# Terence-23/RayTracing-in-a-weekend

Measured on AMD Instinct MI355X. Metric: Msamples/s (rays x bounces) at 1920x1080x500spp, higher is better.
Workload: dtype f32

## Files before the change

raytracing-in-a-weekend_amd/csrc/rtw_host.cpp:

```cpp
#include "rtw_host.h"

#include <algorithm>
#include <cfloat>
#include <cmath>
#include <cstring>
#include <limits>

static_assert(sizeof(RtwCamera) == 84 && sizeof(RtwSphere) == 80 && sizeof(RtwTexture) == 16 && sizeof(RtwQuad) == 88, "POD layout");
static_assert(sizeof(RtwInstance) == 48 && sizeof(RtwScene) == 96 && sizeof(RtwParams) == 72 && sizeof(RtwStats) == 160, "POD layout");

namespace rtw {

uint32_t sampler_count(uint32_t sampler, uint32_t samples, uint32_t *s_root) {
    uint32_t root = 0, n = samples;
    if (sampler == RTW_SAMPLER_STRATIFIED) { root = (uint32_t)std::ceil(std::sqrt((float)samples)); n = root * root; }
    else if (sampler == RTW_SAMPLER_CENTRES) { root = (uint32_t)std::floor(std::sqrt((float)samples)); n = root * root; }
    else if (sampler == RTW_SAMPLER_NO_RAND) n = 1;
    if (s_root) *s_root = root;
    return n;
}

namespace {

struct V { float x, y, z; };
// ... 748 lines not shown
            if (!(radii[i] >= 16.0f * r_med) && std::isfinite(radii[i])) break;
            is_big[i] = 1; out.big.push_back(i);
        }
    }
    std::sort(out.big.begin(), out.big.end());

    Builder b;
    Box centres; box_empty(centres);
    float rmin = FLT_MAX, rmax = 0.0f;
    for (uint32_t i = 0; i < n; i++) {
        if (is_big[i]) continue;
        const RtwSphere &s = spheres[i];
        Prim p; p.sphere = i;
        for (int k = 0; k < 3; k++) {
            float c0 = s.center[k] + s.velocity[k] * t_begin;
            float c1 = s.center[k] + s.velocity[k] * t_end;
            float lo = std::min(c0, c1), hi = std::max(c0, c1);
            if (!(lo == lo) || !(hi == hi)) { lo = -FLT_MAX; hi = FLT_MAX; }
            centres.lo[k] = std::min(centres.lo[k], lo); centres.hi[k] = std::max(centres.hi[k], hi);
            p.cen[k] = 0.5f * lo + 0.5f * hi;
            if (!std::isfinite(p.cen[k])) p.cen[k] = 0.0f;
            p.box.lo[k] = std::nextafter(lo - radii[i], -FLT_MAX);
            p.box.hi[k] = std::nextafter(hi + radii[i], FLT_MAX);
        }
        rmin = std::min(rmin, radii[i]); rmax = std::max(rmax, radii[i]);
        b.prims.push_back(p);
    }
    if (b.prims.empty()) return;
    const uint32_t nl = (uint32_t)b.prims.size();
    Box root_box; box_empty(root_box);
    for (const Prim &p : b.prims) box_grow(root_box, p.box);
    float box_abs = 0.0f;
    for (int k = 0; k < 3; k++) box_abs = std::max(box_abs, std::max(std::fabs(root_box.lo[k]), std::fabs(root_box.hi[k])));
    const bool lds_candidate = nl >= 2 && nl - 1 <= RTW_LDS_NODES_MAX && n <= RTW_LDS_GEOM_MAX && box_abs < 30000.0f;
    b.cap = out.depth_cap = opt.depth_cap ? std::max(opt.depth_cap, ceil_log2(nl)) : bvh_depth_cap(nl, n, lds_candidate);
    b.sweep = opt.sweep && nl <= RTW_BVH_OPTIMISE_MAX;
    b.t.resize(nl);
    for (uint32_t i = 0; i < nl; i++) { b.t[i].box = b.prims[i].box; b.t[i].parent = -1; b.t[i].c[0] = b.t[i].c[1] = -1; b.t[i].height = 0; }
    b.t.reserve(2 * (size_t)nl);
    int32_t troot = b.build(0, nl, 0);
    for (uint32_t i = 0; i < nl; i++) b.t[i].box = b.prims[i].box;
    for (int32_t i = (int32_t)b.t.size() - 1; i >= (int32_t)nl; i--) b.refit(i);
    if (opt.reinsert && nl > 2 && nl <= RTW_BVH_OPTIMISE_MAX) b.reinsertion(troot);
    out.nodes.reserve(nl - 1);
    out.root = b.flatten(troot, 0, out.nodes, out.depth);
    double r2 = 0.0;
    for (int k = 0; k < 3; k++) {
        out.centre[k] = 0.5f * centres.lo[k] + 0.5f * centres.hi[k];
        double h = std::max(std::fabs((double)centres.hi[k] - out.centre[k]), std::fabs((double)centres.lo[k] - out.centre[k]));
        r2 += h * h;
        out.abs_max = std::max(out.abs_max, std::max(std::fabs(root_box.lo[k]), std::fabs(root_box.hi[k])));
    }
    out.centre_radius = (float)(std::sqrt(r2) * 1.000001);
    out.r_min = rmin; out.r_max = rmax;

    if (!out.nodes.empty() && out.nodes.size() <= RTW_LDS_NODES_MAX && n <= RTW_LDS_GEOM_MAX && out.abs_max < 30000.0f) {
        out.nodes16.resize(out.nodes.size());
        for (size_t i = 0; i < out.nodes.size(); i++) {
            const BvhNode &a = out.nodes[i]; BvhNode16 &b = out.nodes16[i];
            for (int k = 0; k < 3; k++) {
                b.plane[0][k][0] = half_bits(a.lo0[k], false); b.plane[0][k][1] = half_bits(a.hi0[k], true);
                b.plane[1][k][0] = half_bits(a.lo1[k], false); b.plane[1][k][1] = half_bits(a.hi1[k], true);
            }
            b.c0 = (int16_t)(a.c0 >= 0 ? a.c0 * 32 : a.c0); b.c1 = (int16_t)(a.c1 >= 0 ? a.c1 * 32 : a.c1); b.pad = 0;
        }
    }
}

void pack_nodes32(const std::vector<BvhNode16> &nodes16, std::vector<uint32_t> &out) {
    const uint32_t AX = RTW_NODE32_AXIS_DWORDS, ND = RTW_NODE32_DWORDS;
    out.assign(nodes16.size() * ND, 0u);
    auto widen = [](uint16_t h) { _Float16 v; std::memcpy(&v, &h, 2); const float f = (float)v; uint32_t u; std::memcpy(&u, &f, 4); return u; };
    auto code = [](int16_t c) { return (uint32_t)(uint16_t)(c >= 0 ? (c / 32) * (int)RTW_NODE32_CODE : (int)c); };
    for (size_t i = 0; i < nodes16.size(); i++) {
        const BvhNode16 &a = nodes16[i];
        uint32_t *d = out.data() + i * ND;
        for (int c = 0; c < 2; c++) for (int k = 0; k < 3; k++) {
            const uint32_t lo = widen(a.plane[c][k][0]), hi = widen(a.plane[c][k][1]);
            uint32_t *q = d + (size_t)(c * 3 + k) * AX;
            q[0] = hi; q[1] = lo; q[2] = lo; q[3] = hi;
        }
        const uint32_t cc = code(a.c0) | (code(a.c1) << 16);
        d[6u * AX] = cc; d[6u * AX + RTW_NODE32_OFF / 4u] = cc;
    }
}

}

namespace rtw {
namespace {
inline float half_value(uint16_t x) { _Float16 v; std::memcpy(&v, &x, 2); return (float)v; }
inline void host_sphere(const RtwSphere &s, uint32_t idx, const float o[3], const float d[3], float tm, float a, float mint, float maxt, int32_t &best, float &best_t) {
    float oc[3];
    for (int k = 0; k < 3; k++) oc[k] = o[k] - (s.center[k] + s.velocity[k] * tm);
    const float b = oc[0] * d[0] + oc[1] * d[1] + oc[2] * d[2], c = (oc[0] * oc[0] + oc[1] * oc[1] + oc[2] * oc[2]) - s.radius * s.radius;
    const float disc = b * b - a * c;
    if (!(disc >= 0.0f)) return;
    const float sq = std::sqrt(disc);
    float x = (-b - sq) / a;
    if (x < mint || x > maxt) x = (-b + sq) / a;
    if (x < mint || x > maxt) return;
    if (best < 0 || x < best_t || (x == best_t && (int32_t)idx < best)) { best = (int32_t)idx; best_t = x; }
}
}

HostHit bvh_closest_host(const BvhBuild &bb, const RtwSphere *spheres, uint32_t n, const float o[3], const float d[3], float tm,
                         float mint, float maxt, bool use_tree, std::string *ops) {
    HostHit h; h.sphere = -1; h.t = maxt; h.node_visits = h.leaf_tests = 0;
    const float a = d[0] * d[0] + d[1] * d[1] + d[2] * d[2];
    if (!use_tree) { for (uint32_t i = 0; i < n; i++) host_sphere(spheres[i], i, o, d, tm, a, mint, maxt, h.sphere, h.t); return h; }
    for (uint32_t i : bb.big) host_sphere(spheres[i], i, o, d, tm, a, mint, maxt, h.sphere, h.t);
    if (bb.root == std::numeric_limits<int32_t>::min()) return h;
    const float M = (std::fabs(o[0] - bb.centre[0]) + std::fabs(o[1] - bb.centre[1]) + std::fabs(o[2] - bb.centre[2])) * 1.0001f + bb.centre_radius;
    const float q = (M * M + bb.r_max * bb.r_max) * 1.4305115e-6f;
    const float sq_q = std::sqrt(q) * 1.0001f;
    float rho = std::fmin(q * (bb.r_min > 0.0f ? 1.0f / (2.0f * bb.r_min) : FLT_MAX), sq_q);
    rho = rho * 1.0001f + 4.8e-7f * (std::fabs(o[0]) + std::fabs(o[1]) + std::fabs(o[2]) + bb.abs_max);
    const float tau = sq_q * 1.0002f / std::sqrt(a) + 1e-30f;
    float inv[3], kp[3], km[3];
    for (int k = 0; k < 3; k++) {
        inv[k] = std::fabs(d[k]) >= 1e-20f ? 1.0f / d[k] : std::copysign(1e20f, d[k]);
        kp[k] = -(o[k] + rho) * inv[k]; km[k] = -(o[k] - rho) * inv[k];
    }
    const float lo_lim = mint - tau;
    const bool f16 = !bb.nodes16.empty();
    std::vector<int32_t> stack; stack.reserve(RTW_BVH_STACK + 2);
    int32_t node = bb.root;
    for (;;) {
        if (node >= 0) {
            h.node_visits++; if (ops) ops->push_back('N');
            const BvhNode &nd = bb.nodes[(size_t)node];
            float e[2], x[2];
            for (int c = 0; c < 2; c++) {
                e[c] = -FLT_MAX; x[c] = FLT_MAX;
                for (int k = 0; k < 3; k++) {
                    const float lo = f16 ? half_value(bb.nodes16[(size_t)node].plane[c][k][0]) : (c ? nd.lo1[k] : nd.lo0[k]);
                    const float hi = f16 ? half_value(bb.nodes16[(size_t)node].plane[c][k][1]) : (c ? nd.hi1[k] : nd.hi0[k]);
                    const float t1 = std::fma(lo, inv[k], kp[k]), t2 = std::fma(hi, inv[k], km[k]);
                    e[c] = std::fmax(e[c], std::fmin(t1, t2)); x[c] = std::fmin(x[c], std::fmax(t1, t2));
                }
            }
            const float hi_lim = h.t + tau;
            const float m0 = std::fmax(e[0], lo_lim), m1 = std::fmax(e[1], lo_lim);
            const bool h0 = m0 <= std::fmin(x[0], hi_lim), h1 = m1 <= std::fmin(x[1], hi_lim);
            if (h0 && h1) { const bool near0 = m0 <= m1; stack.push_back(near0 ? nd.c1 : nd.c0); node = near0 ? nd.c0 : nd.c1; continue; }
            if (h0 || h1) { node = h0 ? nd.c0 : nd.c1; continue; }
        } else {
            h.leaf_tests++; if (ops) ops->push_back('L');
            const uint32_t s = (uint32_t)~node;
            if (s < n) host_sphere(spheres[s], s, o, d, tm, a, mint, maxt, h.sphere, h.t);
        }
        if (stack.empty()) break;
        node = stack.back(); stack.pop_back();
    }
    return h;
}
}

extern "C" int rtw_bvh_dump(const RtwScene *sc, float t_begin, float t_end, void *nodes, uint32_t node_cap, uint32_t *n_nodes, int32_t *root,
                            uint32_t *depth, uint32_t *depth_cap, uint32_t *big, uint32_t big_cap, uint32_t *n_big, uint16_t *nodes16) {
    using namespace rtw;
    if (!sc || (sc->n_spheres && !sc->spheres)) return RTW_E_INVALID;
    BvhBuild b;
    build_bvh(sc->spheres, sc->n_spheres, t_begin, t_end, b);
    if (n_nodes) *n_nodes = (uint32_t)b.nodes.size();
    if (root) *root = b.root;
// ... 213 lines not shown
```

raytracing-in-a-weekend_amd/csrc/rtw_kernels.hip:

```cpp
#include "rtw_kernels.h"
#include "rtw_mesh.h"
#include <type_traits>

#ifndef RTW_MAX_TRIPS
#define RTW_MAX_TRIPS 0x30000000u
#endif

namespace rtw {


constexpr bool gradient_spec(int spec) { return spec >= 1 && spec <= 3; }
constexpr bool generic_spec(int spec) { return spec == 0 || spec == 7 || spec == 8 || spec == 9 || spec == 10 || spec == 11 || spec == 12; }
constexpr bool light_spec(int spec) { return spec == 9 || spec == 10 || spec == 11; }
constexpr int mixed_spec(int spec) { return spec == 10 ? 1 : spec == 11 ? 2 : 0; }
constexpr bool quat_spec(int spec) { return spec == 11; }
constexpr bool noise_spec(int spec) { return spec == 7; }
constexpr bool tri_spec(int spec) { return spec == 8 || spec == 12; }
constexpr bool mesh_spec(int spec) { return spec == 12; }
template <int SPEC> __device__ __forceinline__ uint32_t integ(const KArgs &A) {
    return (SPEC == 5 || SPEC == 12) ? (uint32_t)RTW_INTEGRATOR_RUST2 : SPEC == 4 ? (uint32_t)RTW_INTEGRATOR_BG_COLOR : !generic_spec(SPEC) ? (uint32_t)RTW_INTEGRATOR_GRADIENT : A.integrator;
}
template <int SPEC> __device__ __forceinline__ uint32_t samp(const KArgs &A) {
    return SPEC == 6 ? (uint32_t)RTW_SAMPLER_STRATIFIED : SPEC == 5 ? (uint32_t)RTW_SAMPLER_CENTRES : !generic_spec(SPEC) ? (uint32_t)RTW_SAMPLER_ROW : A.sampler;
}
// ... 592 lines not shown
            if (MOVING) { w0 = vel[s + 4]; w1 = vel[s + 5]; w2 = vel[s + 6]; w3 = vel[s + 7]; }
        }
        test(g0, v0, s); test(g1, v1, s + 1); test(g2, v2, s + 2); test(g3, v3, s + 3);
    }
    for (; s < n; ++s) test(geom[s], MOVING ? vel[s] : zero, s);
}

#ifndef RTW_GEOM_BRUTE_WAVES
#define RTW_GEOM_BRUTE_WAVES 4
#endif
template <bool MOVING, int SPEC, bool GEOM>
__global__ __launch_bounds__(RTW_BLOCK, GEOM ? RTW_GEOM_BRUTE_WAVES : 1) void render_brute(const KArgs A) {
    bool dead = false, have = false, newpath = false;
    Pixel px; px.ij = px.rng_base = px.s = px.slot = 0;
    Reserve rs; rs.next = rs.end = rs.limit = rs.i0 = rs.k0 = rs.s0 = rs.s1 = rs.slot0 = rs.tries = 0; rs.sub = blockIdx.x & ((1u << A.sub_shift) - 1u);
#ifdef RTW_ENDTIMES
    rs.t_dry = 0ull;
#endif
    Path pt; pt.o = pt.d = pt.L = mk(0, 0, 0); pt.thr = mk(1, 1, 1); pt.tm = 0; pt.k = 0; pt.poison = false; pt.rng.state = 0; pt.rng.inc = 1;
    uint32_t n_seg = 0, n_rays = 0, n_isph = 0, n_quad = 0;
    uint32_t trips = 0; bool aborted = false;
    if constexpr (tri_spec(SPEC)) tri_nodes_begin(A);

    for (;;) {
        if (fetch_pixel(A, !have && !dead, px, dead, rs)) { have = true; newpath = true; }
        if (ballot64(!dead) == 0ull) break;
        if (++trips > RTW_MAX_TRIPS) { aborted = true; break; }
        if (have && newpath) { newpath = false; start_path<SPEC>(A, px, pt); n_rays++; }
        if (have) {
            bool finished;
            if (light_spec(SPEC) ? (A.depth == 0 && (mixed_spec(SPEC) ? A.integrator != RTW_INTEGRATOR_LIGHT_CAST : A.integrator == RTW_INTEGRATOR_LIGHT_BIASED))
                                 : (generic_spec(SPEC) && A.depth == 0 && A.integrator != RTW_INTEGRATOR_NORMAL)) {
                pt.L = (light_spec(SPEC) || A.integrator == RTW_INTEGRATOR_RUST2) ? ld3(A.bg) : mk(0, 0, 0); finished = true;
            } else {
                int best; float best_t;
                closest_brute<MOVING>(A.sc, pt.o, pt.d, pt.tm, A.mint, A.maxt, best, best_t);
                n_seg++;
                if constexpr (light_spec(SPEC)) finished = light_step_brute<MOVING, GEOM, mixed_spec(SPEC), quat_spec(SPEC)>(A, pt, best, best_t, n_seg, n_isph, n_quad);
                else finished = GEOM ? shade_geom<MOVING, SPEC>(A, pt, best, best_t, n_isph, n_quad) : shade<MOVING, SPEC>(A, pt, best, best_t);
            }
            if (finished) {
                if (finish_path<SPEC>(A, px, pt)) have = false;
                else newpath = true;
            }
        }
    }
    if constexpr (tri_spec(SPEC)) tri_nodes_end(A);
    flush_counters(A, n_seg, n_rays, (unsigned long long)n_seg * A.sc.n + n_isph, 0);
    if (GEOM) flush_quads(A, n_quad);
    if (aborted && (threadIdx.x & 63u) == 0) atomicAdd(&A.stats[23], 1ull);
}


template <bool MOVING>
__device__ __forceinline__ void exact_sphere(f4 g, f4 vv, uint32_t s, v3 o, v3 d, float tm, float a, float ra, bool a_plain, float mint, float maxt,
                                             int &best, float &best_t) {
    float cx = g.x, cy = g.y, cz = g.z;
    if (MOVING) { cx = cx + vv.x * tm; cy = cy + vv.y * tm; cz = cz + vv.z * tm; }
    float ocx = o.x - cx, ocy = o.y - cy, ocz = o.z - cz;
    float b = ocx * d.x + ocy * d.y + ocz * d.z;
    float c = (ocx * ocx + ocy * ocy + ocz * ocz) - g.w;
    float disc = b * b - a * c;
    if (!(disc < 0.0f)) {
        const float x = sphere_root(b, disc, a, ra, a_plain, mint);
        const bool take = !(x < mint || x > maxt) && (x < best_t || (x == best_t && s < (uint32_t)best));
        best = take ? (int)s : best; best_t = take ? x : best_t;
    }
}

#define RTW_KU 1.4305115e-6f
#ifndef RTW_S_HI
#define RTW_S_HI 52u
#endif
#ifndef RTW_TRAV_UNROLL
#define RTW_TRAV_UNROLL 3
#endif
#ifndef RTW_T_LO
#define RTW_T_LO 6u
#endif
#ifndef RTW_T_LO_DRAIN
#define RTW_T_LO_DRAIN RTW_T_LO
#endif

struct Trav {
    int node;
    uint32_t sp;
    int best; float best_t;
    float a, ra;
    float ix, iy, iz;
    float kpx, kpy, kpz;
    float kmx, kmy, kmz;
    uint32_t selx, sely, selz;
    float tau_t, lo_lim, hi_lim;
};

template <class S> struct Code;
template <> struct Code<short> { enum : int { END = 0x7FFF, DEAD = 0x7FFE }; };
template <> struct Code<int> { enum : int { END = 0x7FFFFFFF, DEAD = 0x7FFFFFFE }; };
template <class S> __device__ __forceinline__ bool in_trav(int node) { return (uint32_t)node < (uint32_t)Code<S>::DEAD; }
template <class S> __device__ __forceinline__ bool in_leaf(int node) { return (uint32_t)node > (uint32_t)Code<S>::END; }
template <class S> __device__ __forceinline__ uint32_t leaf_sphere(int node) { return (uint32_t)node ^ (sizeof(S) == 2 ? 0xFFFFu : 0xFFFFFFFFu); }
template <class S> __device__ __forceinline__ bool in_shade(int node) { return node == (int)Code<S>::END; }

__device__ __forceinline__ uint32_t lanes_in(bool c) {
    uint32_t n = (uint32_t)__popcll(ballot64(c));
    asm volatile("" : "+s"(n));
    return n;
}

struct BvhBegin {
    const f4 *big_geom; const f4 *big_vel; const uint32_t *big_index;
    uint32_t n_big, depth; int32_t root;
    float cx, cy, cz, centre_radius, r_max2, inv_2rmin, abs_max;
};
static_assert(sizeof(BvhBegin) == 64 && offsetof(DevBvh, abs_max) - offsetof(DevBvh, big_geom) == 60 && offsetof(DevBvh, big_vel) == offsetof(DevBvh, big_geom) + 8 &&
              offsetof(DevBvh, n_big) == offsetof(DevBvh, big_geom) + 24 && offsetof(DevBvh, root) == offsetof(DevBvh, big_geom) + 32 &&
              offsetof(DevBvh, cx) == offsetof(DevBvh, big_geom) + 36, "BvhBegin mirrors DevBvh from big_geom on");
__device__ __forceinline__ BvhBegin load_bvh_begin() {
    typedef uint32_t u16v __attribute__((ext_vector_type(16)));
    u16v r;
    asm volatile("s_load_dwordx16 %0, %1, %2\n\ts_waitcnt lgkmcnt(0)" : "=s"(r) : "s"(__builtin_amdgcn_kernarg_segment_ptr()),
                 "n"(offsetof(KArgs, bvh) + offsetof(DevBvh, big_geom)));
    BvhBegin b;
    b.big_geom = (const f4 *)(uintptr_t)((uint64_t)r[0] | ((uint64_t)r[1] << 32));
    b.big_vel = (const f4 *)(uintptr_t)((uint64_t)r[2] | ((uint64_t)r[3] << 32));
    b.big_index = (const uint32_t *)(uintptr_t)((uint64_t)r[4] | ((uint64_t)r[5] << 32));
    b.n_big = r[6]; b.depth = r[7]; b.root = (int32_t)r[8];
    b.cx = __uint_as_float(r[9]); b.cy = __uint_as_float(r[10]); b.cz = __uint_as_float(r[11]); b.centre_radius = __uint_as_float(r[12]);
    b.r_max2 = __uint_as_float(r[13]); b.inv_2rmin = __uint_as_float(r[14]); b.abs_max = __uint_as_float(r[15]);
    return b;
}

template <class T> __device__ __forceinline__ T lds_get(uint32_t addr) { return *(const __attribute__((address_space(3))) T *)(uintptr_t)addr; }
template <class T> __device__ __forceinline__ void lds_put(uint32_t addr, T v) { *(__attribute__((address_space(3))) T *)(uintptr_t)addr = v; }
__device__ __forceinline__ uint32_t lds_addr(const void *p) { return (uint32_t)(uintptr_t)(const __attribute__((address_space(3))) void *)p; }

template <bool MOVING, class S, bool F32 = false>
__device__ __forceinline__ void trav_begin(const KArgs &A, const Path &pt, Trav &tr, uint32_t sp0, bool a_plain_wave, bool &a_odd, Cen *cn = nullptr) {
    RTW_CEN(cn, CEN_TRAV_BEGIN);
    const BvhBegin bv = load_bvh_begin();
    const v3 o = pt.o, d = pt.d;
    tr.a = dot(d, d);
    tr.ra = rcp_refined(tr.a);
    a_odd = !in_range(tr.a, 0x1p-20f, 0x1p20f);
    const bool a_plain = a_plain_wave && ballot64(a_odd) == 0ull;
    tr.best = -1; tr.best_t = A.maxt; tr.sp = sp0;
    {
        cf4_ptr bg = (cf4_ptr)(uintptr_t)bv.big_geom;
        cf4_ptr bvel = (cf4_ptr)(uintptr_t)bv.big_vel;
        typedef const uint32_t __attribute__((address_space(4))) *cu32_ptr;
        cu32_ptr bidx = (cu32_ptr)(uintptr_t)bv.big_index;
        for (uint32_t k = 0; k < bv.n_big; ++k) {
            f4 vv = MOVING ? bvel[k] : f4{ 0, 0, 0, 0 };
            exact_sphere<MOVING>(bg[k], vv, bidx[k], o, d, pt.tm, tr.a, tr.ra, a_plain, A.mint, A.maxt, tr.best, tr.best_t);
        }
    }
    if (bv.root == (int)0x80000000) { tr.node = (int)Code<S>::END; return; }
    tr.node = sizeof(S) == 2 ? (bv.root >= 0 ? bv.root * (F32 ? (int)RTW_NODE32_CODE : 32) : (int)((uint32_t)bv.root & 0xFFFFu)) : bv.root;
    const float ex = o.x - bv.cx, ey = o.y - bv.cy, ez = o.z - bv.cz;
#ifdef RTW_BEGIN_L2_NORM
    const float M = __builtin_amdgcn_sqrtf(ex * ex + ey * ey + ez * ez) * 1.0001f + bv.centre_radius;
#else
    const float M = (__builtin_fabsf(ex) + __builtin_fabsf(ey) + __builtin_fabsf(ez)) * 1.0001f + bv.centre_radius;
#endif
    const float q = (M * M + bv.r_max2) * RTW_KU;
    const float sq_q = __builtin_amdgcn_sqrtf(q) * 1.0001f;
    float rho = fminf(q * bv.inv_2rmin, sq_q);
    rho = rho * 1.0001f + 4.8e-7f * (fabsf(o.x) + fabsf(o.y) + fabsf(o.z) + bv.abs_max);
    tr.tau_t = sq_q * 1.0002f * __builtin_amdgcn_rsqf(tr.a) + 1e-30f;
    float ix = __builtin_amdgcn_rcpf(d.x), iy = __builtin_amdgcn_rcpf(d.y), iz = __builtin_amdgcn_rcpf(d.z);
#ifdef RTW_BEGIN_GUARD_PER_LANE
    if (!(fabsf(d.x) >= 1e-20f)) ix = copysignf(1e20f, d.x);
    if (!(fabsf(d.y) >= 1e-20f)) iy = copysignf(1e20f, d.y);
    if (!(fabsf(d.z) >= 1e-20f)) iz = copysignf(1e20f, d.z);
#else
    if (ballot64(!(fminf(fminf(fabsf(d.x), fabsf(d.y)), fabsf(d.z)) >= 1e-20f) || d.x != d.x || d.y != d.y || d.z != d.z) != 0ull) {
        if (!(fabsf(d.x) >= 1e-20f)) ix = copysignf(1e20f, d.x);
        if (!(fabsf(d.y) >= 1e-20f)) iy = copysignf(1e20f, d.y);
        if (!(fabsf(d.z) >= 1e-20f)) iz = copysignf(1e20f, d.z);
    }
#endif
    tr.ix = ix; tr.iy = iy; tr.iz = iz;
    if (sizeof(S) == 2) {
        const float ox = -o.x * ix, oy = -o.y * iy, oz = -o.z * iz;
        const float rx = rho * fabsf(ix), ry = rho * fabsf(iy), rz = rho * fabsf(iz);
        tr.kpx = ox - rx; tr.kpy = oy - ry; tr.kpz = oz - rz;
        tr.kmx = ox + rx; tr.kmy = oy + ry; tr.kmz = oz + rz;
        const uint32_t ID = 0x03020100u, FLIP = 0x03020100u ^ 0x01000302u;
        if (F32) {
            tr.selx = ~(uint32_t)((int32_t)__float_as_uint(ix) >> 31) & RTW_NODE32_OFF;
            tr.sely = ~(uint32_t)((int32_t)__float_as_uint(iy) >> 31) & RTW_NODE32_OFF;
            tr.selz = ~(uint32_t)((int32_t)__float_as_uint(iz) >> 31) & RTW_NODE32_OFF;
        } else {
        tr.selx = ID ^ ((uint32_t)((int32_t)__float_as_uint(ix) >> 31) & FLIP);
        tr.sely = ID ^ ((uint32_t)((int32_t)__float_as_uint(iy) >> 31) & FLIP);
        tr.selz = ID ^ ((uint32_t)((int32_t)__float_as_uint(iz) >> 31) & FLIP);
        }
    } else {
        tr.kpx = -(o.x + rho) * ix; tr.kpy = -(o.y + rho) * iy; tr.kpz = -(o.z + rho) * iz;
        tr.kmx = -(o.x - rho) * ix; tr.kmy = -(o.y - rho) * iy; tr.kmz = -(o.z - rho) * iz;
    }
    tr.lo_lim = A.mint - tr.tau_t;
    tr.hi_lim = tr.best_t + tr.tau_t;
}


template <class S, uint32_t BLOCK = RTW_BLOCK>
__device__ __forceinline__ void trav_pop(Trav &tr) {
    tr.node = (int)(uint32_t)lds_get<typename std::make_unsigned<S>::type>(tr.sp);
    tr.sp -= BLOCK * (uint32_t)sizeof(S);
}

template <class S> __device__ __forceinline__ int entry_to_node(uint32_t raw);
template <> __device__ __forceinline__ int entry_to_node<short>(uint32_t raw) { return (int)(raw & 0xFFFFu); }
template <> __device__ __forceinline__ int entry_to_node<int>(uint32_t raw) { return (int)raw; }

template <class S, uint32_t BLOCK = RTW_BLOCK>
__device__ __forceinline__ void trav_descend(Trav &tr, float e0, float x0, float e1, float x1,
                                             uint32_t c0, uint32_t c1, uint32_t popped) {
    const float n0 = fmaxf(e0, tr.lo_lim), n1 = fmaxf(e1, tr.lo_lim);
    const bool h0 = n0 <= fminf(x0, tr.hi_lim);
    const bool h1 = n1 <= fminf(x1, tr.hi_lim);
    const bool le = n0 <= n1;
    const bool both = h0 && h1, none = !(h0 || h1);
    const bool near0 = h0 && (!h1 || le);
    const uint32_t level = BLOCK * (uint32_t)sizeof(S);
    if (sizeof(S) == 2) {
        const uint64_t H0 = __builtin_amdgcn_ballot_w64(h0), H1 = __builtin_amdgcn_ballot_w64(h1), LE = __builtin_amdgcn_ballot_w64(le);
        const bool far0 = __builtin_amdgcn_inverse_ballot_w64(~H0 | (H1 & ~LE));
        const uint32_t nf = __builtin_amdgcn_alignbit(c0, c0, far0 ? 16u : 0u);
        lds_put<unsigned short>(tr.sp + level, (unsigned short)(nf >> 16));
        tr.node = entry_to_node<S>(none ? popped : nf);
    } else {
        lds_put<S>(tr.sp + level, (S)(near0 ? c1 : c0));
        tr.node = entry_to_node<S>(none ? popped : (near0 ? c0 : c1));
    }
    tr.sp = (tr.sp + (both ? level : 0u)) - (none ? level : 0u);
}

typedef unsigned int u4 __attribute__((ext_vector_type(4)));
typedef unsigned int u3 __attribute__((ext_vector_type(3)));
typedef unsigned int u32a2 __attribute__((aligned(2)));
__device__ __forceinline__ float h_lo(unsigned int w) { return (float)__builtin_bit_cast(_Float16, (unsigned short)(w & 0xFFFFu)); }
__device__ __forceinline__ float h_hi(unsigned int w) { return (float)__builtin_bit_cast(_Float16, (unsigned short)(w >> 16)); }

__device__ __forceinline__ void trav_node_lds(const u4 *lnodes, Trav &tr) {
    const uint32_t popped = lds_get<unsigned short>(tr.sp);
    const uint32_t at = (uint32_t)tr.node;
    const u4 r0 = lds_get<u4>(at);
    const u3 r1 = lds_get<u3>(at + 16u);
#ifdef RTW_LDS_PROBE
    {
        const uint32_t pa = (uint32_t)tr.node * 32u + ((tr.selx & 1u) << RTW_LDS_PROBE_SH);
        #pragma unroll
        for (int k = 0; k < RTW_LDS_PROBE; k++) { const uint32_t x = lds_get<u32a2>(pa + 4u * k); asm volatile("" :: "v"(x)); }
    }
#endif
    const uint32_t c0 = r1.z, c1 = 0;
    const uint32_t ax = __builtin_amdgcn_perm(r0.x, r0.x, tr.selx), ay = __builtin_amdgcn_perm(r0.y, r0.y, tr.sely), az = __builtin_amdgcn_perm(r0.z, r0.z, tr.selz);
    const uint32_t bx = __builtin_amdgcn_perm(r0.w, r0.w, tr.selx), by = __builtin_amdgcn_perm(r1.x, r1.x, tr.sely), bz = __builtin_amdgcn_perm(r1.y, r1.y, tr.selz);
    const float e0 = fmaxf(fmaxf(__builtin_fmaf(h_lo(ax), tr.ix, tr.kpx), __builtin_fmaf(h_lo(ay), tr.iy, tr.kpy)), __builtin_fmaf(h_lo(az), tr.iz, tr.kpz));
    const float x0 = fminf(fminf(__builtin_fmaf(h_hi(ax), tr.ix, tr.kmx), __builtin_fmaf(h_hi(ay), tr.iy, tr.kmy)), __builtin_fmaf(h_hi(az), tr.iz, tr.kmz));
    const float e1 = fmaxf(fmaxf(__builtin_fmaf(h_lo(bx), tr.ix, tr.kpx), __builtin_fmaf(h_lo(by), tr.iy, tr.kpy)), __builtin_fmaf(h_lo(bz), tr.iz, tr.kpz));
    const float x1 = fminf(fminf(__builtin_fmaf(h_hi(bx), tr.ix, tr.kmx), __builtin_fmaf(h_hi(by), tr.iy, tr.kmy)), __builtin_fmaf(h_hi(bz), tr.iz, tr.kmz));
    trav_descend<short>(tr, e0, x0, e1, x1, c0, c1, popped);
}

typedef float f2a __attribute__((ext_vector_type(2), aligned(RTW_NODE32_OFF)));
__device__ __forceinline__ f2a lds_get_pair(uint32_t addr) { return *(const volatile __attribute__((address_space(3))) f2a *)(uintptr_t)addr; }
template <uint32_t BLOCK>
__device__ __forceinline__ void trav_node_lds32(Trav &tr) {
    const uint32_t popped = lds_get<unsigned short>(tr.sp);
    constexpr uint32_t G = RTW_NODE32_AXIS_DWORDS * 4u;
    const uint32_t ax = ((uint32_t)tr.node << RTW_NODE32_UNIT_SHIFT) + tr.selx, ay = ((uint32_t)tr.node << RTW_NODE32_UNIT_SHIFT) + tr.sely,
                   az = ((uint32_t)tr.node << RTW_NODE32_UNIT_SHIFT) + tr.selz;
    const f2a px0 = lds_get_pair(ax), py0 = lds_get_pair(ay + G), pz0 = lds_get_pair(az + 2u * G);
    const f2a px1 = lds_get_pair(ax + 3u * G), py1 = lds_get_pair(ay + 4u * G), pz1 = lds_get_pair(az + 5u * G);
    const uint32_t c0 = lds_get<uint32_t>(ax + 6u * G), c1 = 0;
    const float e0 = fmaxf(fmaxf(__builtin_fmaf(px0.x, tr.ix, tr.kpx), __builtin_fmaf(py0.x, tr.iy, tr.kpy)), __builtin_fmaf(pz0.x, tr.iz, tr.kpz));
    const float x0 = fminf(fminf(__builtin_fmaf(px0.y, tr.ix, tr.kmx), __builtin_fmaf(py0.y, tr.iy, tr.kmy)), __builtin_fmaf(pz0.y, tr.iz, tr.kmz));
    const float e1 = fmaxf(fmaxf(__builtin_fmaf(px1.x, tr.ix, tr.kpx), __builtin_fmaf(py1.x, tr.iy, tr.kpy)), __builtin_fmaf(pz1.x, tr.iz, tr.kpz));
    const float x1 = fminf(fminf(__builtin_fmaf(px1.y, tr.ix, tr.kmx), __builtin_fmaf(py1.y, tr.iy, tr.kmy)), __builtin_fmaf(pz1.y, tr.iz, tr.kmz));
    trav_descend<short, BLOCK>(tr, e0, x0, e1, x1, c0, c1, popped);
}

__device__ __forceinline__ void trav_node(const DevBvh &bv, Trav &tr) {
    const uint32_t popped = lds_get<uint32_t>(tr.sp);
    const f4 *np = (const f4 *)(bv.nodes + tr.node);
    const f4 n0 = np[0], n1 = np[1], n2 = np[2];
    const uint32_t c0 = (uint32_t)bv.nodes[tr.node].c0, c1 = (uint32_t)bv.nodes[tr.node].c1;
    float t1, t2;
    t1 = __builtin_fmaf(n0.x, tr.ix, tr.kpx); t2 = __builtin_fmaf(n0.w, tr.ix, tr.kmx);
    float e0 = fminf(t1, t2), x0 = fmaxf(t1, t2);
    t1 = __builtin_fmaf(n0.y, tr.iy, tr.kpy); t2 = __builtin_fmaf(n1.x, tr.iy, tr.kmy);
    e0 = fmaxf(e0, fminf(t1, t2)); x0 = fminf(x0, fmaxf(t1, t2));
    t1 = __builtin_fmaf(n0.z, tr.iz, tr.kpz); t2 = __builtin_fmaf(n1.y, tr.iz, tr.kmz);
    e0 = fmaxf(e0, fminf(t1, t2)); x0 = fminf(x0, fmaxf(t1, t2));
    t1 = __builtin_fmaf(n1.z, tr.ix, tr.kpx); t2 = __builtin_fmaf(n2.y, tr.ix, tr.kmx);
    float e1 = fminf(t1, t2), x1 = fmaxf(t1, t2);
    t1 = __builtin_fmaf(n1.w, tr.iy, tr.kpy); t2 = __builtin_fmaf(n2.z, tr.iy, tr.kmy);
    e1 = fmaxf(e1, fminf(t1, t2)); x1 = fminf(x1, fmaxf(t1, t2));
    t1 = __builtin_fmaf(n2.x, tr.iz, tr.kpz); t2 = __builtin_fmaf(n2.w, tr.iz, tr.kmz);
    e1 = fmaxf(e1, fminf(t1, t2)); x1 = fminf(x1, fmaxf(t1, t2));
    trav_descend<int>(tr, e0, x0, e1, x1, c0, c1, popped);
}

#ifdef RTW_STAMP
#define RTW_SUB_STAMP(k) do { asm volatile("s_waitcnt vmcnt(0) lgkmcnt(0)" ::: "memory"); const unsigned long long t_now = __builtin_amdgcn_s_memtime(); sub[k] += t_now - t_sub; t_sub = t_now; } while (0)
#else
#define RTW_SUB_STAMP(k) do { } while (0)
#endif
#ifndef RTW_BVH_WAVES
#define RTW_BVH_WAVES 4
#endif
template <bool MOVING, class S>
__device__ __forceinline__ void wild_ray_query(const KArgs &A, const Path &pt, Trav &tr, uint32_t &n_tests) {
    const float m = (__builtin_fabsf(pt.o.x) + __builtin_fabsf(pt.o.y) + __builtin_fabsf(pt.o.z)) +
                    (__builtin_fabsf(pt.d.x) + __builtin_fabsf(pt.d.y) + __builtin_fabsf(pt.d.z));
    if (m < 0x1p60f) return;
    closest_brute<MOVING>(A.sc, pt.o, pt.d, pt.tm, A.mint, A.maxt, tr.best, tr.best_t);
    tr.node = (int)Code<S>::END;
    n_tests += A.sc.n - A.bvh.n_big;
}

#ifndef RTW_BVH_WAVES_GEOM
#define RTW_BVH_WAVES_GEOM 2
#endif
#ifndef RTW_BVH_WAVES_GEOM_SPEC
#define RTW_BVH_WAVES_GEOM_SPEC 5
#endif
#ifndef RTW_BVH_WAVES_SPEC
#define RTW_BVH_WAVES_SPEC 7
#endif
#ifndef RTW_BVH_WAVES_SPEC2
#define RTW_BVH_WAVES_SPEC2 RTW_BVH_WAVES_SPEC
#endif
#ifndef RTW_BVH_WAVES_FOLDED
#define RTW_BVH_WAVES_FOLDED RTW_BVH_WAVES
#endif
constexpr bool two_halves_step(int spec, bool geom, bool moving) {
#ifdef RTW_NO_TWO_HALVES
    return false;
#else
    return gradient_spec(spec) && !geom && !(moving && spec == 2);
#endif
}
constexpr uint32_t bvh_block(bool moving, int nodes, int spec, bool geom) {
    return !moving && !geom && nodes == 1 && two_halves_step(spec, geom, moving) ? RTW_BLOCK_LARGE : RTW_BLOCK;
}
template <bool MOVING, int NODES, int SPEC, bool GEOM>
__global__ __launch_bounds__(bvh_block(MOVING, NODES, SPEC, GEOM), GEOM ? (!generic_spec(SPEC) ? RTW_BVH_WAVES_GEOM_SPEC : RTW_BVH_WAVES_GEOM) : (two_halves_step(SPEC, GEOM, MOVING) ? (SPEC == 2 ? RTW_BVH_WAVES_SPEC2 : RTW_BVH_WAVES_SPEC) : (gradient_spec(SPEC) ? RTW_BVH_WAVES_SPEC2 : (!generic_spec(SPEC) ? RTW_BVH_WAVES_FOLDED : RTW_BVH_WAVES)))) void render_bvh(const KArgs A) {
    constexpr bool LDSN = NODES != 0, geom_in_lds = NODES == 2;
    constexpr uint32_t BLOCK = bvh_block(MOVING, NODES, SPEC, GEOM);
    constexpr bool F32 = BLOCK != RTW_BLOCK;
    typedef typename std::conditional<LDSN, short, int>::type stack_t;
    extern __shared__ __attribute__((aligned(16))) unsigned char lds_raw[];
    *(stack_t *)(lds_raw + A.lds_stack_off + threadIdx.x * (uint32_t)sizeof(stack_t)) = (stack_t)Code<stack_t>::END;
    u4 *lnodes = (u4 *)lds_raw;
    if (LDSN && lds_addr(lds_raw) != 0u) { if (threadIdx.x == 0) atomicAdd(&A.stats[23], 1ull); return; }
    f4 *lgeom = (f4 *)(lds_raw + A.lds_geom_off);
    const DevScene &sc = A.sc;
    if (LDSN) {
        const u4 *src = F32 ? (const u4 *)A.nodes32 : (const u4 *)A.bvh.nodes16;
        const uint32_t n16 = A.bvh.n_nodes * (F32 ? RTW_NODE32_DWORDS / 4u : 2u);
        for (uint32_t i = threadIdx.x; i < n16; i += BLOCK) lnodes[i] = src[i];
        if (geom_in_lds) for (uint32_t i = threadIdx.x; i < sc.n; i += BLOCK) lgeom[i] = sc.geom[i];
        __syncthreads();
    }
    if constexpr (tri_spec(SPEC)) tri_nodes_begin(A);

    enum : uint32_t { F_HAVE = 1u,
                      F_INFLIGHT = 2u,
                      F_NEWPATH = 4u,
                      F_DONE = 8u,
                      F_K_SHIFT = 8u };
    uint32_t fl = 0u;
    Pixel px; px.ij = px.rng_base = px.s = px.slot = 0;
    Reserve rs; rs.next = rs.end = rs.limit = rs.i0 = rs.k0 = rs.s0 = rs.s1 = rs.slot0 = rs.tries = 0; rs.sub = blockIdx.x & ((1u << A.sub_shift) - 1u);
#ifdef RTW_ENDTIMES
    rs.t_dry = 0ull;
#endif
    Path pt; pt.o = pt.d = pt.L = mk(0, 0, 0); pt.thr = mk(1, 1, 1); pt.tm = 0; pt.k = 0; pt.poison = false; pt.rng.state = 0; pt.rng.inc = 1;
    typename std::conditional<light_spec(SPEC), LightPath, char>::type lp{};
    Trav tr; tr.node = (int)Code<stack_t>::END; tr.sp = 0; tr.best = -1; tr.best_t = 0; tr.a = tr.ra = 1; tr.ix = tr.iy = tr.iz = 0;
    tr.kpx = tr.kpy = tr.kpz = tr.kmx = tr.kmy = tr.kmz = 0; tr.selx = tr.sely = tr.selz = 0; tr.tau_t = tr.lo_lim = tr.hi_lim = 0;
    uint32_t w_seg = 0, w_rays = 0;
    uint32_t t_lo = RTW_T_LO;
    uint32_t trips = 0; bool aborted = false;
    bool a_plain = true;
    uint32_t n_isph = 0, n_quad = 0;
    uint32_t c_steps[3] = { 0, 0, 0 };
    uint32_t c_lanes[3] = { 0, 0, 0 };
#ifdef RTW_STAMP
    unsigned long long c_time[3] = { 0, 0, 0 };
    unsigned long long sub[5] = { 0, 0, 0, 0, 0 }, t_sub = 0;
#endif
#ifdef RTW_CENSUS
    Cen cen_store; for (int k = 0; k < CEN_N; k++) cen_store.n[k] = cen_store.w[k] = 0u;
    Cen *const cn = &cen_store;
#else
    Cen *const cn = nullptr;
#endif

#ifdef RTW_ENDTIMES
    const unsigned long long t_wave_start = __builtin_amdgcn_s_memtime();
    const unsigned long long rt_wave_start = wall_clock64();
    uint32_t dry_trips = 0, dry_steps[3] = { 0, 0, 0 }, dry_lanes[3] = { 0, 0, 0 };
    uint32_t dry_queries = 0;
#endif
    for (;;) {
        uint32_t nT = lanes_in(in_trav<stack_t>(tr.node));
        const uint32_t nL = lanes_in(in_leaf<stack_t>(tr.node));
        const uint32_t nS = lanes_in(in_shade<stack_t>(tr.node));
        if ((nT | nL | nS) == 0u) break;
        if (++trips > RTW_MAX_TRIPS) { aborted = true; break; }
        RTW_CEN(cn, CEN_BIG_ROOT);
        const bool run_shade = nS >= RTW_S_HI || (nT < t_lo && nL < t_lo && nS > 0u);
        const bool run_leaf = nL > nT;
#ifdef RTW_ENDTIMES
        if (rs.t_dry) {
            dry_trips++;
            const int ph = run_shade ? 2 : (run_leaf ? 1 : 0);
            dry_steps[ph]++; dry_lanes[ph] += ph == 2 ? nS : (ph == 1 ? nL : nT);
            if (run_shade && in_shade<stack_t>(tr.node) && (fl & F_INFLIGHT)) dry_queries++;
        }
#endif
#ifdef RTW_STAMP
        const unsigned long long t_begin = __builtin_amdgcn_s_memtime();
        const int which = run_shade ? 2 : (run_leaf ? 1 : 0);
#endif
        bool burst = false;
        if (run_shade) {
            c_steps[2]++; c_lanes[2] += nS;
            bool need_unit = false, started = false, a_odd = false;
            const bool shading = in_shade<stack_t>(tr.node);
            w_seg += (uint32_t)__popcll(ballot64(shading && (fl & F_INFLIGHT) != 0u));
#ifdef RTW_STAMP
            t_sub = t_begin;
#endif
            if constexpr (two_halves_step(SPEC, GEOM, MOVING)) {
            bool need_ball = false, need_disk = false, front = false;
            v3 nrm, ud; float metal;
            bool hit = false;
            if (shading) {
                RTW_CEN(cn, CEN_SHADING);
                if (fl & F_INFLIGHT) {
                    fl &= ~F_INFLIGHT;
                    RTW_CEN(cn, CEN_INFLIGHT);
                    ud = unit(pt.d);
                    if (tr.best < 0) { RTW_CEN(cn, CEN_MISS); fl |= F_DONE; }
                    else if ((fl >> F_K_SHIFT) + 1u >= A.depth) { RTW_CEN(cn, CEN_DEPTH_END); fl |= F_DONE; }
                    else { hit = true; fl += 1u << F_K_SHIFT; }
                }
            }
            RTW_SUB_STAMP(0);
            if (shading) {
                if (fl & F_DONE) {
                    fl &= ~F_DONE;
                    if (tr.best < 0) shade_miss<SPEC>(A, pt, ud); else pt.L = mk(0, 0, 0);
                    if (finish_path<SPEC>(A, px, pt, cn)) fl &= ~F_HAVE; else fl |= F_NEWPATH;
                }
                need_unit = (fl & F_HAVE) == 0u;
                if (need_unit) RTW_CEN(cn, CEN_NEED_UNIT);
            }
            bool exhausted = false;
            const bool got = fetch_pixel(A, need_unit, px, exhausted, rs);
            if (ballot64(exhausted) != 0ull) t_lo = RTW_T_LO_DRAIN;
            RTW_SUB_STAMP(1);
            if (shading) {
                if (got) fl |= F_HAVE | F_NEWPATH;
                if (exhausted) tr.node = (int)Code<stack_t>::DEAD;
                if ((fl & F_HAVE) && (fl & F_NEWPATH)) { fl &= F_HAVE | F_INFLIGHT | F_DONE; start_path_first(px, pt, cn); need_disk = true; started = true; }
            }
            if (hit) shade_hit_first<MOVING, SPEC>(A, pt, ud, tr.best, tr.best_t, need_ball, nrm, metal, front, cn);
            float sx, sy, sz, sl2;
            sample_ball_or_disk(pt.rng, need_ball || need_disk, need_ball, sx, sy, sz, sl2, cn);
            if (need_ball) pt.d = on_hit_second(metal, nrm, pt.d, front, mk(sx, sy, sz), sl2);
            if (need_disk) start_path_second(px, pt, sx, sy);
            RTW_SUB_STAMP(2);
            if (shading && (fl & F_HAVE)) {
                trav_begin<MOVING, stack_t, F32>(A, pt, tr, lds_addr(lds_raw) + A.lds_stack_off + threadIdx.x * (uint32_t)sizeof(stack_t), a_plain, a_odd, cn);
                fl |= F_INFLIGHT;
            }
            RTW_SUB_STAMP(3);
            } else {
            if (shading) {
                RTW_CEN(cn, CEN_SHADING);
                if (fl & F_INFLIGHT) {
                    fl &= ~F_INFLIGHT;
                    bool done;
                    if constexpr (light_spec(SPEC)) done = light_step_bvh<MOVING, GEOM, mixed_spec(SPEC), quat_spec(SPEC)>(A, pt, lp, fl, tr.best, tr.best_t, n_isph, n_quad);
                    else done = GEOM ? shade_geom<MOVING, SPEC>(A, pt, tr.best, tr.best_t, n_isph, n_quad) : shade<MOVING, SPEC>(A, pt, tr.best, tr.best_t, cn);
                    if (done) fl |= F_DONE;
                }
            }
            RTW_SUB_STAMP(0);
            if (shading) {
                if (fl & F_DONE) { fl &= ~F_DONE; if (finish_path<SPEC>(A, px, pt, cn)) fl &= ~F_HAVE; else fl |= F_NEWPATH; }
                need_unit = (fl & F_HAVE) == 0u;
                if (need_unit) RTW_CEN(cn, CEN_NEED_UNIT);
            }
            bool exhausted = false;
            const bool got = fetch_pixel(A, need_unit, px, exhausted, rs);
            if (ballot64(exhausted) != 0ull) t_lo = RTW_T_LO_DRAIN;
            RTW_SUB_STAMP(1);
#ifdef RTW_STAMP
            if (shading) {
                if (got) fl |= F_HAVE | F_NEWPATH;
                if (exhausted) tr.node = (int)Code<stack_t>::DEAD;
                if ((fl & F_HAVE) && (fl & F_NEWPATH)) { fl &= ~F_NEWPATH; start_path<SPEC>(A, px, pt); started = true; }
            }
            RTW_SUB_STAMP(2);
#endif
            if (shading) {
                if (got) fl |= F_HAVE | F_NEWPATH;
                if (exhausted) tr.node = (int)Code<stack_t>::DEAD;
                if (fl & F_HAVE) {
                    if (fl & F_NEWPATH) { fl &= ~F_NEWPATH; start_path<SPEC>(A, px, pt, cn); started = true; }
                    if (light_spec(SPEC) ? (A.depth == 0 && (mixed_spec(SPEC) ? A.integrator != RTW_INTEGRATOR_LIGHT_CAST : A.integrator == RTW_INTEGRATOR_LIGHT_BIASED))
                                         : (generic_spec(SPEC) && A.depth == 0 && A.integrator != RTW_INTEGRATOR_NORMAL)) {
                        pt.L = (light_spec(SPEC) || A.integrator == RTW_INTEGRATOR_RUST2) ? ld3(A.bg) : mk(0, 0, 0);
                        fl |= F_DONE;
                    } else {
                        trav_begin<MOVING, stack_t, F32>(A, pt, tr, lds_addr(lds_raw) + A.lds_stack_off + threadIdx.x * (uint32_t)sizeof(stack_t), a_plain, a_odd, cn);
                        if constexpr (GEOM || light_spec(SPEC)) wild_ray_query<MOVING, stack_t>(A, pt, tr, n_isph);
                        fl |= F_INFLIGHT;
                    }
                }
            }
            RTW_SUB_STAMP(3);
            }
            w_rays += (uint32_t)__popcll(ballot64(started));
            if (ballot64(a_odd) != 0ull) a_plain = false;
#ifndef RTW_STAMP
            nT = lanes_in(in_trav<stack_t>(tr.node)); burst = nT >= 33u;
#endif
        } else {
            burst = !run_leaf;
            if (run_leaf) {
                c_steps[1]++; c_lanes[1] += nL;
                if (in_leaf<stack_t>(tr.node)) {
                    const uint32_t s = leaf_sphere<stack_t>(tr.node);
                    const f4 gs = geom_in_lds ? lgeom[s] : sc.geom[s];
                    exact_sphere<MOVING>(gs, MOVING ? sc.vel[s] : f4{ 0, 0, 0, 0 }, s, pt.o, pt.d, pt.tm, tr.a, tr.ra, a_plain, A.mint, A.maxt, tr.best, tr.best_t);
                    tr.hi_lim = tr.best_t + tr.tau_t;
                    trav_pop<stack_t, BLOCK>(tr);
                }
#ifndef RTW_STAMP
                nT = lanes_in(in_trav<stack_t>(tr.node)); burst = nT >= 33u;
#endif
            }
        }
        if (burst) {
            static_assert(RTW_S_HI > 31u && RTW_T_LO <= 33u, "the shortcut below assumes the thresholds of the scheduler");
            uint32_t live = nT;
            for (;;) {
                uint32_t b_steps = 0, b_lanes = 0;
                for (int u = 0; u < RTW_TRAV_UNROLL; u++) {
                    b_steps++; b_lanes += live;
                    if (in_trav<stack_t>(tr.node)) {
                        if constexpr (F32) trav_node_lds32<BLOCK>(tr);
                        else if (LDSN) trav_node_lds((const u4 *)lnodes, tr); else trav_node(A.bvh, tr);
                    }
                    if (u + 1 >= RTW_TRAV_UNROLL) break;
                    live = lanes_in(in_trav<stack_t>(tr.node));
                    if (live == 0u) break;
                }
                asm volatile("" : "+s"(b_steps), "+s"(b_lanes));
                c_steps[0] += b_steps; c_lanes[0] += b_lanes;
#ifdef RTW_STAMP
                break;
#else
                if (live == 0u) break;
                live = lanes_in(in_trav<stack_t>(tr.node));
                if (live < 33u) break;
                if (++trips > RTW_MAX_TRIPS) break;
#endif
            }
        }
#ifdef RTW_STAMP
        asm volatile("s_waitcnt vmcnt(0) lgkmcnt(0)" ::: "memory");
        c_time[which] += __builtin_amdgcn_s_memtime() - t_begin;
#endif
    }
    if constexpr (tri_spec(SPEC)) tri_nodes_end(A);
    if (GEOM || light_spec(SPEC)) { flush_quads(A, n_quad); flush_tests(A, n_isph); }
#ifdef RTW_CENSUS
    for (int k = 0; k < CEN_N; k++) {
        unsigned long long w = cn->w[k], n = cn->n[k];
        for (int off = 32; off > 0; off >>= 1) { w += __shfl_down(w, off); n += __shfl_down(n, off); }
        if ((threadIdx.x & 63u) == 0) { atomicAdd(&A.stats[32 + 2 * k], w); atomicAdd(&A.stats[33 + 2 * k], n); }
    }
#endif
#ifdef RTW_ENDTIMES
    uint32_t dry_q_max = dry_queries, dry_q_sum = dry_queries;
    for (int off = 32; off > 0; off >>= 1) { const uint32_t o = __shfl_down(dry_q_max, off); dry_q_max = o > dry_q_max ? o : dry_q_max; dry_q_sum += __shfl_down(dry_q_sum, off); }
#endif
    if ((threadIdx.x & 63u) == 0) {
        atomicAdd(&A.stats[0], (unsigned long long)w_rays);
        atomicAdd(&A.stats[1], (unsigned long long)w_seg);
        atomicAdd(&A.stats[2], (unsigned long long)c_lanes[1] + (unsigned long long)w_seg * A.bvh.n_big);
        atomicAdd(&A.stats[3], (unsigned long long)c_lanes[0]);
        for (int k = 0; k < 3; k++) { atomicAdd(&A.stats[5 + k], (unsigned long long)c_steps[k]); atomicAdd(&A.stats[8 + k], (unsigned long long)c_lanes[k]); }
        if (aborted) atomicAdd(&A.stats[23], 1ull);
#ifdef RTW_STAMP
        for (int k = 0; k < 3; k++) atomicAdd(&A.stats[11 + k], c_time[k]);
        for (int k = 0; k < 4; k++) atomicAdd(&A.stats[16 + k], sub[k]);
#endif
#ifdef RTW_ENDTIMES
        const unsigned long long t_end = __builtin_amdgcn_s_memtime();
        atomicMax(&A.stats[12], t_end - t_wave_start);
        if (A.endtimes_ref) {
            const unsigned long long bin = (t_end - t_wave_start) * 32ull / A.endtimes_ref;
            const unsigned long long b = bin >= 32ull ? 11ull : (bin >= 21ull ? bin - 21ull : 0ull);
            atomicAdd(&A.stats[20 + b], 1ull);
        }
        atomicAdd(&A.stats[13], t_end - t_wave_start);
        atomicAdd(&A.stats[15], 1ull);
        const unsigned long long rt_end = wall_clock64();
        atomicMin(&A.stats[24 + 8 - 8], rt_wave_start + 0ull);
        atomicMax(&A.stats[25], rt_wave_start);
        atomicMin(&A.stats[26], rt_end);
        atomicMax(&A.stats[27], rt_end);
        if (rs.t_dry) { atomicMin(&A.stats[28], rs.t_dry); atomicMax(&A.stats[29], rs.t_dry); atomicMax(&A.stats[30], rt_end - rs.t_dry); atomicAdd(&A.stats[31], rt_end - rs.t_dry); }
        if (rs.t_dry && rt_end - rs.t_dry >= 60000ull) {
            atomicAdd(&A.stats[40], 1ull); atomicAdd(&A.stats[41], rt_end - rs.t_dry); atomicAdd(&A.stats[42], (unsigned long long)dry_trips);
            for (int k = 0; k < 3; k++) { atomicAdd(&A.stats[43 + k], (unsigned long long)dry_steps[k]); atomicAdd(&A.stats[46 + k], (unsigned long long)dry_lanes[k]); }
            atomicAdd(&A.stats[49], (unsigned long long)dry_q_max); atomicAdd(&A.stats[50], (unsigned long long)dry_q_sum);
        }
#endif
    }
}

template <int SPEC, bool GEOM>
static render_fn kernel_of(bool bvh, bool moving, int nodes) {
    if (!bvh) return moving ? render_brute<true, SPEC, GEOM> : render_brute<false, SPEC, GEOM>;
    if (nodes == 0) return moving ? render_bvh<true, 0, SPEC, GEOM> : render_bvh<false, 0, SPEC, GEOM>;
    if (nodes == 1) return moving ? render_bvh<true, 1, SPEC, GEOM> : render_bvh<false, 1, SPEC, GEOM>;
    if constexpr (!GEOM) if (nodes == 2) return moving ? render_bvh<true, 2, SPEC, false> : render_bvh<false, 2, SPEC, false>;
    return nullptr;
}
render_fn render_kernel(const RenderBuild &b) {
    if (!b.bvh && b.nodes != 0) return nullptr;
    switch (b.spec * 2 + (b.geom ? 1 : 0)) {
#define RTW_BUILD(SPEC, GEOM) case SPEC * 2 + GEOM: return kernel_of<SPEC, GEOM != 0>(b.bvh, b.moving, b.nodes);
    RTW_BUILD(0, 0) RTW_BUILD(1, 0) RTW_BUILD(2, 0) RTW_BUILD(3, 0) RTW_BUILD(4, 0) RTW_BUILD(5, 0) RTW_BUILD(6, 0) RTW_BUILD(7, 0) RTW_BUILD(9, 0) RTW_BUILD(10, 0)
    RTW_BUILD(0, 1) RTW_BUILD(2, 1) RTW_BUILD(4, 1) RTW_BUILD(5, 1) RTW_BUILD(6, 1) RTW_BUILD(7, 1) RTW_BUILD(8, 1) RTW_BUILD(9, 1) RTW_BUILD(10, 1) RTW_BUILD(11, 1) RTW_BUILD(12, 1)
#undef RTW_BUILD
    default: return nullptr;
    }
}

uint32_t render_block(const RenderBuild &b) { return b.bvh ? bvh_block(b.moving, b.nodes, b.spec, b.geom) : RTW_BLOCK; }

void launch_render(render_fn fn, uint32_t block, const KArgs &a, uint32_t grid, hipStream_t stream) {
    hipLaunchKernelGGL(fn, dim3(grid), dim3(block), a.lds_bytes, stream, a);
    hipLaunchKernelGGL(resolve_kernel, dim3((a.n_tiles * 64u + RTW_BLOCK - 1) / RTW_BLOCK), dim3(RTW_BLOCK), 0, stream, a);
}
// ... 68 lines not shown
```

Baseline: 40650.

## Add per-block-size scheduler thresholds and store swapped child codes for f32 nodes

Adds a compile-time Sched table so the large-block (f32 LDS node) kernel variant uses its own thresholds for shading, draining and traversal bursts: lower chain threshold and higher t_lo. For f32 nodes the host now also stores a half-swapped child code word, so the kernel reads both words with one paired LDS load and picks near/far with a select instead of alignbit. This aims to keep SIMD lanes busier in traversal bursts and trim an ALU op per node, at the cost of running bursts at lower lane occupancy and one extra LDS dword per node.

Result: faster. 41750 (median of 6 runs) (+2.7%).

```diff
diff --git a/raytracing-in-a-weekend_amd/csrc/rtw_host.cpp b/raytracing-in-a-weekend_amd/csrc/rtw_host.cpp
--- a/raytracing-in-a-weekend_amd/csrc/rtw_host.cpp
+++ b/raytracing-in-a-weekend_amd/csrc/rtw_host.cpp
@@ -854,6 +854,8 @@
         }
         const uint32_t cc = code(a.c0) | (code(a.c1) << 16);
         d[6u * AX] = cc; d[6u * AX + RTW_NODE32_OFF / 4u] = cc;
+        const uint32_t sw = (cc >> 16) | (cc << 16);
+        d[6u * AX + 1u] = sw; d[6u * AX + RTW_NODE32_OFF / 4u + 1u] = sw;
     }
 }
 
diff --git a/raytracing-in-a-weekend_amd/csrc/rtw_kernels.hip b/raytracing-in-a-weekend_amd/csrc/rtw_kernels.hip
--- a/raytracing-in-a-weekend_amd/csrc/rtw_kernels.hip
+++ b/raytracing-in-a-weekend_amd/csrc/rtw_kernels.hip
@@ -698,6 +698,27 @@
 #define RTW_T_LO_DRAIN RTW_T_LO
 #endif
 
+#ifndef RTW_CHAIN
+#define RTW_CHAIN 33u
+#endif
+#ifndef RTW_S_HI_LARGE
+#define RTW_S_HI_LARGE RTW_S_HI
+#endif
+#ifndef RTW_T_LO_LARGE
+#define RTW_T_LO_LARGE 8u
+#endif
+#ifndef RTW_TRAV_UNROLL_LARGE
+#define RTW_TRAV_UNROLL_LARGE RTW_TRAV_UNROLL
+#endif
+#ifndef RTW_CHAIN_LARGE
+#define RTW_CHAIN_LARGE 13u
+#endif
+struct Sched { uint32_t s_hi, t_lo, t_lo_drain; int burst; uint32_t chain; };
+constexpr Sched sched_of(uint32_t block) {
+    return block == RTW_BLOCK_LARGE ? Sched{ RTW_S_HI_LARGE, RTW_T_LO_LARGE, RTW_T_LO_LARGE, RTW_TRAV_UNROLL_LARGE, RTW_CHAIN_LARGE }
+                                    : Sched{ RTW_S_HI, RTW_T_LO, RTW_T_LO_DRAIN, RTW_TRAV_UNROLL, RTW_CHAIN };
+}
+
 struct Trav {
     int node;
     uint32_t sp;
@@ -844,7 +865,9 @@
     if (sizeof(S) == 2) {
         const uint64_t H0 = __builtin_amdgcn_ballot_w64(h0), H1 = __builtin_amdgcn_ballot_w64(h1), LE = __builtin_amdgcn_ballot_w64(le);
         const bool far0 = __builtin_amdgcn_inverse_ballot_w64(~H0 | (H1 & ~LE));
-        const uint32_t nf = __builtin_amdgcn_alignbit(c0, c0, far0 ? 16u : 0u);
+        uint32_t nf;
+        if constexpr (BLOCK != RTW_BLOCK) nf = far0 ? c1 : c0;
+        else nf = __builtin_amdgcn_alignbit(c0, c0, far0 ? 16u : 0u);
         lds_put<unsigned short>(tr.sp + level, (unsigned short)(nf >> 16));
         tr.node = entry_to_node<S>(none ? popped : nf);
     } else {
@@ -892,7 +915,8 @@
                    az = ((uint32_t)tr.node << RTW_NODE32_UNIT_SHIFT) + tr.selz;
     const f2a px0 = lds_get_pair(ax), py0 = lds_get_pair(ay + G), pz0 = lds_get_pair(az + 2u * G);
     const f2a px1 = lds_get_pair(ax + 3u * G), py1 = lds_get_pair(ay + 4u * G), pz1 = lds_get_pair(az + 5u * G);
-    const uint32_t c0 = lds_get<uint32_t>(ax + 6u * G), c1 = 0;
+    const f2a cc = lds_get_pair(ax + 6u * G);
+    const uint32_t c0 = __float_as_uint(cc.x), c1 = __float_as_uint(cc.y);
     const float e0 = fmaxf(fmaxf(__builtin_fmaf(px0.x, tr.ix, tr.kpx), __builtin_fmaf(py0.x, tr.iy, tr.kpy)), __builtin_fmaf(pz0.x, tr.iz, tr.kpz));
     const float x0 = fminf(fminf(__builtin_fmaf(px0.y, tr.ix, tr.kmx), __builtin_fmaf(py0.y, tr.iy, tr.kmy)), __builtin_fmaf(pz0.y, tr.iz, tr.kmz));
     const float e1 = fmaxf(fmaxf(__builtin_fmaf(px1.x, tr.ix, tr.kpx), __builtin_fmaf(py1.x, tr.iy, tr.kpy)), __builtin_fmaf(pz1.x, tr.iz, tr.kpz));
@@ -969,6 +993,7 @@
     constexpr bool LDSN = NODES != 0, geom_in_lds = NODES == 2;
     constexpr uint32_t BLOCK = bvh_block(MOVING, NODES, SPEC, GEOM);
     constexpr bool F32 = BLOCK != RTW_BLOCK;
+    constexpr Sched SC = sched_of(BLOCK);
     typedef typename std::conditional<LDSN, short, int>::type stack_t;
     extern __shared__ __attribute__((aligned(16))) unsigned char lds_raw[];
     *(stack_t *)(lds_raw + A.lds_stack_off + threadIdx.x * (uint32_t)sizeof(stack_t)) = (stack_t)Code<stack_t>::END;
@@ -1001,7 +1026,7 @@
     Trav tr; tr.node = (int)Code<stack_t>::END; tr.sp = 0; tr.best = -1; tr.best_t = 0; tr.a = tr.ra = 1; tr.ix = tr.iy = tr.iz = 0;
     tr.kpx = tr.kpy = tr.kpz = tr.kmx = tr.kmy = tr.kmz = 0; tr.selx = tr.sely = tr.selz = 0; tr.tau_t = tr.lo_lim = tr.hi_lim = 0;
     uint32_t w_seg = 0, w_rays = 0;
-    uint32_t t_lo = RTW_T_LO;
+    uint32_t t_lo = SC.t_lo;
     uint32_t trips = 0; bool aborted = false;
     bool a_plain = true;
     uint32_t n_isph = 0, n_quad = 0;
@@ -1031,7 +1056,7 @@
         if ((nT | nL | nS) == 0u) break;
         if (++trips > RTW_MAX_TRIPS) { aborted = true; break; }
         RTW_CEN(cn, CEN_BIG_ROOT);
-        const bool run_shade = nS >= RTW_S_HI || (nT < t_lo && nL < t_lo && nS > 0u);
+        const bool run_shade = nS >= SC.s_hi || (nT < t_lo && nL < t_lo && nS > 0u);
         const bool run_leaf = nL > nT;
 #ifdef RTW_ENDTIMES
         if (rs.t_dry) {
@@ -1081,7 +1106,7 @@
             }
             bool exhausted = false;
             const bool got = fetch_pixel(A, need_unit, px, exhausted, rs);
-            if (ballot64(exhausted) != 0ull) t_lo = RTW_T_LO_DRAIN;
+            if (ballot64(exhausted) != 0ull) t_lo = SC.t_lo_drain;
             RTW_SUB_STAMP(1);
             if (shading) {
                 if (got) fl |= F_HAVE | F_NEWPATH;
@@ -1118,7 +1143,7 @@
             }
             bool exhausted = false;
             const bool got = fetch_pixel(A, need_unit, px, exhausted, rs);
-            if (ballot64(exhausted) != 0ull) t_lo = RTW_T_LO_DRAIN;
+            if (ballot64(exhausted) != 0ull) t_lo = SC.t_lo_drain;
             RTW_SUB_STAMP(1);
 #ifdef RTW_STAMP
             if (shading) {
@@ -1149,7 +1174,7 @@
             w_rays += (uint32_t)__popcll(ballot64(started));
             if (ballot64(a_odd) != 0ull) a_plain = false;
 #ifndef RTW_STAMP
-            nT = lanes_in(in_trav<stack_t>(tr.node)); burst = nT >= 33u;
+            nT = lanes_in(in_trav<stack_t>(tr.node)); burst = nT >= SC.chain;
 #endif
         } else {
             burst = !run_leaf;
@@ -1163,22 +1188,22 @@
                     trav_pop<stack_t, BLOCK>(tr);
                 }
 #ifndef RTW_STAMP
-                nT = lanes_in(in_trav<stack_t>(tr.node)); burst = nT >= 33u;
+                nT = lanes_in(in_trav<stack_t>(tr.node)); burst = nT >= SC.chain;
 #endif
             }
         }
         if (burst) {
-            static_assert(RTW_S_HI > 31u && RTW_T_LO <= 33u, "the shortcut below assumes the thresholds of the scheduler");
+            static_assert(SC.s_hi > 64u - SC.chain && SC.t_lo <= SC.chain, "the shortcut below assumes the thresholds of the scheduler");
             uint32_t live = nT;
             for (;;) {
                 uint32_t b_steps = 0, b_lanes = 0;
-                for (int u = 0; u < RTW_TRAV_UNROLL; u++) {
+                for (int u = 0; u < SC.burst; u++) {
                     b_steps++; b_lanes += live;
                     if (in_trav<stack_t>(tr.node)) {
                         if constexpr (F32) trav_node_lds32<BLOCK>(tr);
                         else if (LDSN) trav_node_lds((const u4 *)lnodes, tr); else trav_node(A.bvh, tr);
                     }
-                    if (u + 1 >= RTW_TRAV_UNROLL) break;
+                    if (u + 1 >= SC.burst) break;
                     live = lanes_in(in_trav<stack_t>(tr.node));
                     if (live == 0u) break;
                 }
@@ -1189,7 +1214,7 @@
 #else
                 if (live == 0u) break;
                 live = lanes_in(in_trav<stack_t>(tr.node));
-                if (live < 33u) break;
+                if (live < SC.chain) break;
                 if (++trips > RTW_MAX_TRIPS) break;
 #endif
             }
```
